# vismaychuriwala/Fast-Image-Editing-with-Generative-Models

Measured on AMD Instinct MI355X. Metric: PIE-Bench images/sec @1024^2 SSD-1B fp16 4-step, higher is better.
Workload: dtype f16

## Files before the change

### fast-image-editing-with-generative-models_amd/csrc/conv_halo.hip

```cpp
#include "gemm_common.h"

using namespace fie_gemm;

namespace {

constexpr int HP = 18;
constexpr int HPIECES = (HP * HP + 7) / 8;
constexpr int HALO_B = HPIECES * 1024;
constexpr int HSLOTS = 6;
constexpr int BNH = 128;
constexpr int STH = 3;
constexpr int WSTAGE_B = BNH * 128;
constexpr int WRING_OFF = 0;
constexpr int HALO_OFF = STH * WSTAGE_B;
constexpr int DUMP_OFF = HALO_OFF + 2 * HALO_B;
constexpr int kLdsHalo = DUMP_OFF + 1024;
constexpr int RWH = BNH / 64;

constexpr int n_w(bool last, int t) { return last && t + 2 > 8 ? 0 : RWH; }
constexpr int n_h(bool last, int t) { return !last && t < HSLOTS ? 1 : 0; }
constexpr int n_wait(bool last, int t) { return (t > 0 ? n_h(last, t - 1) : 0) + n_w(last, t) + n_h(last, t); }

template <bool STAMP>
__global__ __launch_bounds__(512) void conv_halo_kernel(GemmArgs p) {
    constexpr int FM = 4, FN = 4, WM = 64, WN = 64;
    extern __shared__ __attribute__((aligned(16))) half_t smem[];
    char* const lds = reinterpret_cast<char*>(smem);

    const int tid = threadIdx.x;
    const int lane = tid & 63;
    const int wave = __builtin_amdgcn_readfirstlane(tid >> 6);
    const int grp = wave >> 2;
    const int wm = wave & 3, wn = wave >> 2;

    const int bid = xcd_remap(blockIdx.x, gridDim.x);
    const int nt = bid % p.nbn, patch = bid / p.nbn;
    const int ppr = p.OW >> 4, ppi = (p.OH >> 4) * ppr;
    const int b = patch / ppi, pr = patch - b * ppi;
    const int py = pr / ppr, px = pr - py * ppr;
    const int y0 = py << 4, x0 = px << 4;
    const int m0 = (b * p.OH + y0) * p.OW + x0, n0 = nt * BNH;

    const int live = p.probe == 1 ? 0 : 1;
    const __amdgpu_buffer_rsrc_t rs_a = buf_rsrc(p.A1, (int)p.a1_bytes * live);
    const __amdgpu_buffer_rsrc_t rs_w = buf_rsrc(p.Wt, (int)p.w_bytes * live);

    unsigned h_off[HSLOTS];
#pragma unroll
    for (int i = 0; i < HSLOTS; ++i) {
        const int q = wave + 8 * i;
        const int pl = q * 8 + (lane >> 3);
        const int hy = pl / HP, hx = pl - hy * HP;
        const int iy = y0 + hy - 1, ix = x0 + hx - 1;
        const bool ok = q < HPIECES && pl < HP * HP && iy >= 0 && iy < p.H && ix >= 0 && ix < p.W;
        const unsigned chunk = (unsigned)((lane & 7) ^ (hx & 7));
        h_off[i] = ok ? ((unsigned)(b * p.H + iy) * (unsigned)p.W + (unsigned)ix) * (unsigned)p.Cin * 2u + chunk * 16u : kOob;
    }
    auto halo_dst = [&](int i, int buf) -> half_t* {
        const int q = wave + 8 * i;
        return reinterpret_cast<half_t*>(lds + (q < HPIECES ? HALO_OFF + buf * HALO_B + q * 1024 : DUMP_OFF));
    };
    const int lr = lane >> 3;
    const unsigned w_base = (unsigned)(n0 + wave * 8 + lr) * (unsigned)p.ldw * 2u + (unsigned)((lane & 7) ^ lr) * 16u;
    const unsigned w_step = 64u * (unsigned)p.ldw * 2u;
    auto issue_w = [&](int stage, unsigned soff) {
#pragma unroll
        for (int i = 0; i < RWH; ++i)
            bload16(rs_w, reinterpret_cast<half_t*>(lds + WRING_OFF + stage * WSTAGE_B + (wave + 8 * i) * 1024), w_base + (unsigned)i * w_step, soff);
    };
    const unsigned cin2 = (unsigned)p.Cin * 2u;

    const int fr = lane & 15, fq = lane >> 4;
    unsigned a_rd[3][2];
#pragma unroll
    for (int kx = 0; kx < 3; ++kx)
#pragma unroll
        for (int kh = 0; kh < 2; ++kh)
            a_rd[kx][kh] = (unsigned)((wm * FM * HP + fr + kx) * 128 + (((kh * 4 + fq) ^ ((fr + kx) & 7)) << 4));
    unsigned w_rd[2];
#pragma unroll
    for (int kh = 0; kh < 2; ++kh) w_rd[kh] = (unsigned)(2 * lds_off(wn * WN + fr, kh * 4 + fq));

    f32x4 acc[FN][FM];
#pragma unroll
    for (int i = 0; i < FN; ++i)
#pragma unroll
        for (int j = 0; j < FM; ++j) acc[i][j] = (f32x4){0.f, 0.f, 0.f, 0.f};

    unsigned seg[8] = {0, 0, 0, 0, 0, 0, 0, 0}, tprev = 0;
    auto stamp = [&](int i) {
        if constexpr (STAMP) {
            __builtin_amdgcn_sched_barrier(0);
            const unsigned t = (unsigned)__builtin_amdgcn_s_memtime();
            seg[i] += t - tprev;
            tprev = t;
            __builtin_amdgcn_sched_barrier(0);
        }
    };
    if constexpr (STAMP) tprev = (unsigned)__builtin_amdgcn_s_memtime();

    const int nchunks = p.Cin / BK;
#pragma unroll
    for (int i = 0; i < HSLOTS; ++i) bload16(rs_a, halo_dst(i, 0), h_off[i], 0u);
    issue_w(0, 0u);
    issue_w(1, nchunks * 9 > 1 ? cin2 : 0u);
    wait_vm_barrier<RWH>();
    if (grp == 1) __builtin_amdgcn_s_barrier();
    stamp(5);

    f16x8 fw[2][FN], fa[2][FM];
    auto kstep = [&](auto lastc, auto tapc, int c, unsigned hb) {
        constexpr bool LAST = decltype(lastc)::value;
        constexpr int T = decltype(tapc)::value;
        constexpr int KY = T / 3, KX = T % 3;
        constexpr int STAGE = T % STH, FILL = (T + 2) % STH;
        if constexpr (n_w(LAST, T) > 0) {
            constexpr int T2 = (T + 2) % 9;
            const int c2 = T + 2 > 8 ? c + 1 : c;
            issue_w(FILL, (unsigned)T2 * cin2 + (unsigned)c2 * (BK * 2));
        }
        if constexpr (n_h(LAST, T) > 0) bload16(rs_a, halo_dst(T, (c + 1) & 1), h_off[T], (unsigned)(c + 1) * (BK * 2));
        stamp(0);
        const char* const hal = lds + HALO_OFF + hb;
        const char* const wst = lds + WRING_OFF + STAGE * WSTAGE_B;
#pragma unroll
        for (int kh = 0; kh < 2; ++kh) {
#pragma unroll
            for (int i = 0; i < FN; ++i) fw[kh][i] = *reinterpret_cast<const f16x8*>(wst + w_rd[kh] + i * 16 * 128);
#pragma unroll
            for (int j = 0; j < FM; ++j) fa[kh][j] = *reinterpret_cast<const f16x8*>(hal + a_rd[KX][kh] + (j + KY) * HP * 128);
        }
        asm volatile("s_waitcnt lgkmcnt(0)" ::: "memory");
        stamp(1);
        wait_vm_barrier<n_wait(LAST, T)>();
        stamp(2);
        __builtin_amdgcn_sched_barrier(0);
        __builtin_amdgcn_s_setprio(1);
#pragma unroll
        for (int kh = 0; kh < 2; ++kh)
#pragma unroll
            for (int i = 0; i < FN; ++i)
#pragma unroll
                for (int j = 0; j < FM; ++j) acc[i][j] = __builtin_amdgcn_mfma_f32_16x16x32_f16(fw[kh][i], fa[kh][j], acc[i][j], 0, 0, 0);
        __builtin_amdgcn_s_setprio(0);
        __builtin_amdgcn_sched_barrier(0);
        stamp(3);
        __builtin_amdgcn_s_barrier();
        stamp(4);
    };
    auto chunk = [&](auto lastc, int c) {
        const unsigned hb = (c & 1) ? (unsigned)HALO_B : 0u;
        kstep(lastc, std::integral_constant<int, 0>{}, c, hb);
        kstep(lastc, std::integral_constant<int, 1>{}, c, hb);
        kstep(lastc, std::integral_constant<int, 2>{}, c, hb);
        kstep(lastc, std::integral_constant<int, 3>{}, c, hb);
        kstep(lastc, std::integral_constant<int, 4>{}, c, hb);
        kstep(lastc, std::integral_constant<int, 5>{}, c, hb);
        kstep(lastc, std::integral_constant<int, 6>{}, c, hb);
        kstep(lastc, std::integral_constant<int, 7>{}, c, hb);
        kstep(lastc, std::integral_constant<int, 8>{}, c, hb);
    };
    for (int c = 0; c + 1 < nchunks; ++c) chunk(std::false_type{}, c);
    chunk(std::true_type{}, nchunks - 1);
    if (grp == 0) __builtin_amdgcn_s_barrier();

    epilogue<FM, FN, WM, WN, true, true>(p, acc, m0, n0, wm, wn, lane);
    if constexpr (STAMP) {
        asm volatile("s_waitcnt vmcnt(0)" ::: "memory");
        stamp(6);
        if (p.stamps && lane == 0) {
#pragma unroll
            for (int i = 0; i < 8; ++i) p.stamps[((size_t)bid * 8 + wave) * 8 + i] = seg[i];
        }
    }
}


constexpr int K_FIRST = 0, K_MID = 1, K_LAST_F = 2, K_LAST_N = 3, K_LASTREG_S = 4;
constexpr int n2_w(int kind, int t) { return kind == K_LAST_N && t + 2 > 8 ? 0 : RWH; }
constexpr int n2_h(int kind, int t) { return kind != K_LAST_N && t < HSLOTS ? 1 : 0; }
constexpr int n2_st(int var, int kind, int t) { return kind == K_FIRST && t < 8 ? ((var & 2) ? 1 : 2) : 0; }
constexpr int n2_tail(bool res, int kind, int t) { return n2_h(kind, t); }
constexpr int n2_wait(int var, bool res, int kind, int t) {
    return (t > 0 ? n2_tail(res, kind, t - 1) : 0) + ((var & 8) ? 0 : n2_w(kind, t) + n2_tail(res, kind, t));
}
static_assert(n2_tail(true, K_LAST_F, 8) == 0 && n2_tail(true, K_FIRST, 8) == 0 && n2_st(0, K_FIRST, 8) == 0, "tap 8 carries nothing behind its weights");

template <bool RES, bool GN, bool RB, int VAR, bool STAMP, bool SIDE = false, bool GNA = false, bool EDGE = false>
__global__ __launch_bounds__(512) void conv_halo2_kernel(GemmArgs p) {
    constexpr int FM = 4, FN = 4, WN = 64;
    constexpr bool ST16 = (VAR & 2) != 0, STM = (VAR & 4) != 0, IM = (VAR & 8) != 0;
    constexpr bool DEFER = ST16 && STM && !IM;
    static_assert(!(SIDE && (RES || RB)), "1x1 side inputs belong to a resnet's conv2 + shortcut: no residual, no row bias");
    static_assert(!EDGE || (ST16 && !GN && !GNA), "edge patches: 16-byte stores, no GroupNorm sums");
    extern __shared__ __attribute__((aligned(16))) half_t smem[];
    char* const lds = reinterpret_cast<char*>(smem);

    const int tid = threadIdx.x;
// ... 606 lines not shown
                    asm volatile("s_nop 1\n\tv_permlane16_swap_b32 %0, %1" : "+v"(v[0]), "+v"(v[2]));
                    asm volatile("s_nop 1\n\tv_permlane16_swap_b32 %0, %1" : "+v"(v[1]), "+v"(v[3]));
                }
                __builtin_amdgcn_raw_buffer_store_b128(v, rs_c, edge_off(ro_prev + (unsigned)(2 * jj) * c_jstep + (unsigned)(i * 32), 2 * jj), 0, 0);
            }
    } else {
#pragma unroll
        for (int j = 0; j < FM; ++j)
#pragma unroll
            for (int i = 0; i < FN; ++i) __builtin_amdgcn_raw_buffer_store_b64(outp[i][j], rs_c, ro_prev + (unsigned)j * c_jstep + (unsigned)(i * 32), 0, 0);
    }
    if constexpr (STAMP) {
        asm volatile("s_waitcnt vmcnt(0)" ::: "memory");
        stamp(6);
        if (p.stamps && lane == 0) {
#pragma unroll
            for (int i = 0; i < 8; ++i) p.stamps[((size_t)bid * 8 + wave) * 12 + i] = seg[i];
#pragma unroll
            for (int i = 0; i < 4; ++i) p.stamps[((size_t)bid * 8 + wave) * 12 + 8 + i] = kseg[i];
        }
    }
}

template <bool RES, bool GN, bool RB, int VAR, bool STAMP, bool SIDE = false, bool GNA = false, bool EDGE = false>
hipError_t halo2_attr() {
    return hipFuncSetAttribute(reinterpret_cast<const void*>(&conv_halo2_kernel<RES, GN, RB, VAR, STAMP, SIDE, GNA, EDGE>), hipFuncAttributeMaxDynamicSharedMemorySize, kLdsHalo);
}

}

int fie_conv_halo_init(void) {
    hipError_t e = hipFuncSetAttribute(reinterpret_cast<const void*>(&conv_halo_kernel<false>), hipFuncAttributeMaxDynamicSharedMemorySize, kLdsHalo);
    if (e == hipSuccess) e = hipFuncSetAttribute(reinterpret_cast<const void*>(&conv_halo_kernel<true>), hipFuncAttributeMaxDynamicSharedMemorySize, kLdsHalo);
    if (e == hipSuccess) e = halo2_attr<false, false, false, 6, false>();
    if (e == hipSuccess) e = halo2_attr<false, true, false, 6, false>();
    if (e == hipSuccess) e = halo2_attr<true, false, false, 6, false>();
    if (e == hipSuccess) e = halo2_attr<true, true, false, 6, false>();
    if (e == hipSuccess) e = halo2_attr<false, false, true, 6, false>();
    if (e == hipSuccess) e = halo2_attr<false, true, true, 6, false>();
    if (e == hipSuccess) e = halo2_attr<false, false, false, 0, false>();
    if (e == hipSuccess) e = halo2_attr<false, true, false, 0, false>();
    if (e == hipSuccess) e = halo2_attr<true, false, false, 0, false>();
    if (e == hipSuccess) e = halo2_attr<true, true, false, 0, false>();
    if (e == hipSuccess) e = halo2_attr<false, false, true, 0, false>();
    if (e == hipSuccess) e = halo2_attr<false, true, true, 0, false>();
    if (e == hipSuccess) e = halo2_attr<false, false, false, 6, true>();
    if (e == hipSuccess) e = hipFuncSetAttribute(reinterpret_cast<const void*>(&conv_halo2_kernel<false, false, false, 6, false, true>), hipFuncAttributeMaxDynamicSharedMemorySize, kLdsHalo);
    if (e == hipSuccess) e = hipFuncSetAttribute(reinterpret_cast<const void*>(&conv_halo2_kernel<false, true, false, 6, false, true>), hipFuncAttributeMaxDynamicSharedMemorySize, kLdsHalo);
    if (e == hipSuccess) e = halo2_attr<true, true, false, 6, true>();
    if (e == hipSuccess) e = hipFuncSetAttribute(reinterpret_cast<const void*>(&conv_halo2_kernel<false, true, false, 6, false, false, true>), hipFuncAttributeMaxDynamicSharedMemorySize, kLdsHalo + 8192);
    if (e == hipSuccess) e = hipFuncSetAttribute(reinterpret_cast<const void*>(&conv_halo2_kernel<true, true, false, 6, false, false, true>), hipFuncAttributeMaxDynamicSharedMemorySize, kLdsHalo + 8192);
    if (e == hipSuccess) e = halo2_attr<false, false, false, 6, false, false, false, true>();
    if (e == hipSuccess) e = halo2_attr<true, false, false, 6, false, false, false, true>();
    if (e == hipSuccess) e = halo2_attr<false, false, true, 6, false, false, false, true>();
    if (e == hipSuccess) e = halo2_attr<false, false, false, 6, false, true, false, true>();
    if (e != hipSuccess) {
        fie_set_error("conv_halo: hipFuncSetAttribute failed: %s", hipGetErrorString(e));
        return FIE_EHIP;
    }
    return FIE_OK;
}

bool fie_conv_halo_ok(const GemmArgs& a) {
    const bool base = a.stride == 1 && !a.ups && !a.taps2 && !a.oscat && a.pt == 1 && a.pl == 1 && a.H == a.OH && a.W == a.OW && a.OH % 16 == 0 &&
                      a.OW % 16 == 0 && a.Cin % BK == 0 && a.Cin >= BK && !a.w_scale && !a.out_f8 && a.splitk <= 1;
    if (!base) return false;
    if (!a.A2) return !a.A3 && a.K == 9 * a.Cin;
    return a.C2x % BK == 0 && a.C3x % BK == 0 && a.C2x > 0 && (a.A3 != nullptr) == (a.C3x > 0) && a.K == 9 * a.Cin + a.C2x + a.C3x && a.Cin >= 2 * BK && a.N % BNH == 0 &&
           !a.res && !a.rowbias && a.act == FIE_ACT_NONE && a.scale == 1.f && a.lda2 * 2 * (int64_t)a.OW * a.OH < (1ll << 31) && a.lda3 * 2 * (int64_t)a.OW * a.OH < (1ll << 31);
}

bool fie_conv_halo_edge_ok(const GemmArgs& a) {
    const bool base = a.stride == 1 && !a.ups && !a.taps2 && !a.oscat && a.pt == 1 && a.pl == 1 && a.H == a.OH && a.W == a.OW && a.OH > 0 && a.OW > 0 &&
                      (a.OH % 16 != 0 || a.OW % 16 != 0) && a.M % (a.OH * a.OW) == 0 && a.Cin % BK == 0 && a.Cin >= 2 * BK && !a.w_scale && !a.out_f8 &&
                      a.splitk <= 1 && a.N % 64 == 0 && a.ldc >= a.N && !a.gn_partial && !a.gna_tab && a.act == FIE_ACT_NONE && a.scale == 1.f && !(a.rowbias && a.res);
    if (!base) return false;
    if (!a.A2) return !a.A3 && a.K == 9 * a.Cin;
    return a.C2x % BK == 0 && a.C3x % BK == 0 && a.C2x > 0 && (a.A3 != nullptr) == (a.C3x > 0) && a.K == 9 * a.Cin + a.C2x + a.C3x && !a.res && !a.rowbias &&
           a.lda2 * 2 * (int64_t)a.OW * a.OH < (1ll << 31) && a.lda3 * 2 * (int64_t)a.OW * a.OH < (1ll << 31);
}

int64_t fie_conv_halo_patches(const GemmArgs& a) {
    if (a.OH <= 0 || a.OW <= 0) return 0;
    return (int64_t)(a.M / (a.OH * a.OW)) * ((a.OH + 15) / 16) * ((a.OW + 15) / 16);
}

bool fie_conv_halo_gna_ok(const GemmArgs& a) {
    if (!fie_conv_halo_ok(a) || a.A2 || a.rowbias) return false;
    const int nbn = (a.N + BNH - 1) / BNH;
    return a.M == a.OH * a.OW && a.Cin >= 2 * BK && a.Cin <= 1024 && a.N % BNH == 0 && nbn <= 64 && a.act == FIE_ACT_NONE && a.scale == 1.f && a.gn_partial != nullptr &&
           (a.gn_cg == 4 || a.gn_cg == 8 || a.gn_cg == 16);
}

int fie_launch_conv_halo(fie_ctx* ctx, GemmArgs& a, int variant) {
    if (variant == 6) {
        FIE_REQUIRE(fie_conv_halo_edge_ok(a), "halo-resident conv with edge patches (tile code 78): stride-1 same-size 3x3 conv with H or W %% 16 != 0, Cin %% 64 == 0, "
                    "Cin >= 128, N %% 64 == 0, no activation / scale / GroupNorm sums only");
        a.frag_ld = a.OW;
        a.nbn = (a.N + BNH - 1) / BNH;
        a.nbm = (int)fie_conv_halo_patches(a);
        const int tiles = a.nbm * a.nbn;
        int g = tiles < ctx->num_cus ? tiles : ctx->num_cus;
        g -= g % a.nbn;
        FIE_REQUIRE(g >= a.nbn && a.nbn <= ctx->num_cus, "halo-resident conv: more column tiles than CUs");
        const dim3 grid((unsigned)g);
        if (a.A2) fie_launch(ctx, (conv_halo2_kernel<false, false, false, 6, false, true, false, true>), grid, dim3(512), kLdsHalo, a);
        else if (a.res) fie_launch(ctx, (conv_halo2_kernel<true, false, false, 6, false, false, false, true>), grid, dim3(512), kLdsHalo, a);
        else if (a.rowbias) fie_launch(ctx, (conv_halo2_kernel<false, false, true, 6, false, false, false, true>), grid, dim3(512), kLdsHalo, a);
        else fie_launch(ctx, (conv_halo2_kernel<false, false, false, 6, false, false, false, true>), grid, dim3(512), kLdsHalo, a);
        FIE_LAUNCH_CHECK();
        return FIE_OK;
    }
    FIE_REQUIRE(fie_conv_halo_ok(a), "halo-resident conv: stride-1 same-size 3x3 conv with H, W %% 16 == 0 and Cin %% 64 == 0 only");
    a.frag_ld = a.OW;
    a.nbn = (a.N + BNH - 1) / BNH;
    a.nbm = (a.M / (a.OH * a.OW)) * (a.OH >> 4) * (a.OW >> 4);
    const int tiles = a.nbm * a.nbn;
    const bool side = a.A2 != nullptr;
    FIE_REQUIRE(!(side && variant != 2), "halo-resident conv: 1x1 side inputs run on tile code 72 only");
    if (a.gna_tab) {
        FIE_REQUIRE(fie_conv_halo_gna_ok(a), "halo-resident conv with the input's GroupNorm applied in LDS: shape or epilogue not built (fie_conv3x3_gn_ok)");
        int g = tiles < ctx->num_cus ? tiles : ctx->num_cus;
        g -= g % a.nbn;
        const int lds_bytes = kLdsHalo + a.Cin * 8;
        if (a.res) fie_launch(ctx, (conv_halo2_kernel<true, true, false, 6, false, false, true>), dim3((unsigned)g), dim3(512), lds_bytes, a);
        else fie_launch(ctx, (conv_halo2_kernel<false, true, false, 6, false, false, true>), dim3((unsigned)g), dim3(512), lds_bytes, a);
        FIE_LAUNCH_CHECK();
        return FIE_OK;
    }
    if (!side && variant >= 2 && tiles <= ctx->num_cus) variant = variant == 4 ? 1 : 0;
    if (!side && variant >= 2 && (a.Cin < 2 * BK || a.N % BNH != 0 || (a.rowbias && a.res) || (variant == 4 && a.rowbias) || a.act != FIE_ACT_NONE || a.scale != 1.f)) variant = variant == 4 ? 1 : 0;
    if (variant < 2) {
        const dim3 grid((unsigned)tiles);
        if (variant == 1) fie_launch(ctx, (conv_halo_kernel<true>), grid, dim3(512), kLdsHalo, a);
        else fie_launch(ctx, (conv_halo_kernel<false>), grid, dim3(512), kLdsHalo, a);
        FIE_LAUNCH_CHECK();
        return FIE_OK;
    }
    int g = tiles < ctx->num_cus ? tiles : ctx->num_cus;
    g -= g % a.nbn;
    FIE_REQUIRE(g >= a.nbn && a.nbn <= ctx->num_cus, "halo-resident conv: more column tiles than CUs");
    const dim3 grid((unsigned)g);
    const bool res = a.res != nullptr, gn = a.gn_partial != nullptr, rb = a.rowbias != nullptr;
    FIE_REQUIRE(!gn || a.gn_cg == 4 || a.gn_cg == 8 || a.gn_cg == 16, "halo-resident conv: GroupNorm sums need 4, 8 or 16 channels per group");
#define FIE_HALO2(RES, GN, RB, VAR, ST) fie_launch(ctx, (conv_halo2_kernel<RES, GN, RB, VAR, ST>), grid, dim3(512), kLdsHalo, a)
#define FIE_HALO2_V(VAR)                                                                   \
    do {                                                                                   \
        if (rb && gn) FIE_HALO2(false, true, true, VAR, false);                            \
        else if (rb) FIE_HALO2(false, false, true, VAR, false);                            \
        else if (res && gn) FIE_HALO2(true, true, false, VAR, false);                      \
        else if (res) FIE_HALO2(true, false, false, VAR, false);                           \
        else if (gn) FIE_HALO2(false, true, false, VAR, false);                            \
// ... 12 lines not shown
```

### fast-image-editing-with-generative-models_amd/csrc/gemm_common.h

```cpp
#pragma once
#include "fie_internal.h"
#include "gemm_addr.h"

namespace fie_gemm {

constexpr int BK = 64;

struct GemmArgs {
    const half_t* A1; int64_t lda1; int K1;
    const half_t* A2; int64_t lda2;
    const half_t* A3; int64_t lda3; int C2x, C3x; int64_t a3_bytes;
    int H, W, Cin, OH, OW, stride, pt, pl, ups;
    const half_t* Wt; int64_t ldw;
    half_t* C; int64_t ldc;
    int M, N, K;
    const half_t* bias;
    const half_t* rowbias; int64_t ld_rowbias; int rows_per_batch;
    const half_t* res; int64_t ldr;
    float scale; int act;
    int nbm, nbn;
    int64_t a1_bytes, a2_bytes, w_bytes;
    int taps2, oscat, opy, opx;
    int64_t w_par_stride;
    int gn_nch, gn_chunk0;
// ... 504 lines not shown
    asm volatile("s_waitcnt vmcnt(0)" ::: "memory");
    __syncthreads();
#pragma unroll
    for (int i = 0; i < FN; ++i)
#pragma unroll
        for (int j = 0; j < FM; ++j) acc[i][j] = (f32x4){0.f, 0.f, 0.f, 0.f};
    for (int s = 0; s < S; ++s) {
        const __amdgpu_buffer_rsrc_t rs = buf_rsrc(base + (size_t)s * kTile, kTile * 4);
        u32x4 v[FN][FM];
#pragma unroll
        for (int i = 0; i < FN; ++i)
#pragma unroll
            for (int j = 0; j < FM; ++j) v[i][j] = __builtin_amdgcn_raw_buffer_load_b128(rs, (unsigned)((i * FM + j) * NW * 64 + tid) * 16u, 0, 16);
#pragma unroll
        for (int i = 0; i < FN; ++i)
#pragma unroll
            for (int j = 0; j < FM; ++j) acc[i][j] += __builtin_bit_cast(f32x4, v[i][j]);
    }
    return true;
}

__device__ __forceinline__ int xcd_remap(int bid, int nwg) {
    const int q = nwg >> 3, r = nwg & 7, xcd = bid & 7;
    return (xcd < r ? xcd * (q + 1) : r * (q + 1) + (xcd - r) * q) + (bid >> 3);
}

}

int fie_launch_gemm8(fie_ctx* ctx, const fie_gemm::GemmArgs& a, int conv, int split);
int fie_gemm8_init(void);
int fie_gemm_init(void);
int fie_launch_conv_halo(fie_ctx* ctx, fie_gemm::GemmArgs& a, int stamped);
bool fie_conv_halo_ok(const fie_gemm::GemmArgs& a);
bool fie_conv_halo_edge_ok(const fie_gemm::GemmArgs& a);
int64_t fie_conv_halo_patches(const fie_gemm::GemmArgs& a);
int fie_launch_conv_thin(fie_ctx* ctx, fie_gemm::GemmArgs& a);
bool fie_conv_thin_ok(const fie_gemm::GemmArgs& a);
bool fie_conv_halo_gna_ok(const fie_gemm::GemmArgs& a);
int fie_conv_halo_init(void);
int fie_launch_gemm_w8(fie_ctx* ctx, const fie_gemm::GemmArgs& a, int conv, int code);
int fie_gemm_w8_init(void);
int fie_launch_gemm_x8(fie_ctx* ctx, const fie_gemm::GemmArgs& a, int code, int conv);
int fie_gemm_x8_init(void);
```

### fast-image-editing-with-generative-models_amd/csrc/gemm_conv.hip

```cpp
#include <algorithm>
#include <cstdio>
#include <cstdlib>
#include <cstring>
#include <utility>

#include "gemm_common.h"
#include "gemm_tiles.h"

using namespace fie_gemm;

namespace {

template <int BM, int BN, int MODE>
__global__ __launch_bounds__(256) void gemm_kernel(GemmArgs p) {
    constexpr int WM = BM / 2, WN = BN / 2;
    constexpr int FM = WM / 16, FN = WN / 16;
    constexpr int RA = BM / 32, RW = BN / 32;
    __shared__ __attribute__((aligned(16))) half_t smem[2 * (BM + BN) * BK];

    const int tid = threadIdx.x;
    const int lane = tid & 63, wave = tid >> 6;
    const int wm = wave & 1, wn = wave >> 1;

    const int bid = xcd_remap(blockIdx.x, gridDim.x);
// ... 548 lines not shown
}
template <int BM, int BN>
constexpr Tile generic_row(int code, int w8, int x8) { return {code, BM, BN, kGeneric, "gemm_kernel", 0, w8, x8, &launch_generic<BM, BN, 0>, &launch_generic<BM, BN, 1>}; }
template <int CONV, int VARIANT>
int launch_phased(fie_ctx* ctx, GemmArgs& a, dim3) { return fie_launch_gemm8(ctx, a, CONV, VARIANT); }
template <int VARIANT>
int launch_halo(fie_ctx* ctx, GemmArgs& a, dim3) { return fie_launch_conv_halo(ctx, a, VARIANT); }
int launch_thin(fie_ctx* ctx, GemmArgs& a, dim3) { return fie_launch_conv_thin(ctx, a); }

constexpr Tile kTiles[] = {
    generic_row<128, 128>(1, 62, 43),
    generic_row<128, 64>(2, 42, 42),
    generic_row<64, 64>(3, 43, 43),
    RingTile<128, 64, 3, 4, kSplitK | kLnFold>::row(42, "gemm3_kernel", 42, 42),
    RingTile<64, 64, 3, 4, kSplitK>::row(43, "gemm3_kernel", 43, 43),
    RingTile<128, 64, 2, 4, kSplitK>::row(44, "gemm3_kernel", 42, 42),
    RingTile<64, 64, 2, 4, kSplitK>::row(46, "gemm3_kernel", 43, 43),
    RingTile<128, 96, 3, 4, kSplitK>::row(47, "gemm3_kernel", 62, 47),
    RingTile<128, 80, 3, 4, kSplitK>::row(48, "gemm3_kernel", 62, 0),
    RingTile<128, 128, 3, 8, kSplitK>::row(51, "gemm3_kernel", 62, 51),
    RingTile<128, 128, 2, 8, kSplitK>::row(52, "gemm3_kernel", 52, 52),
    RingTile<192, 128, 2, 8, kSplitK>::row(54, "gemm3_kernel", 54, 54),
    RingTile<256, 256, 2, 8>::row(61, "gemm3_kernel", 62, 62),
    RingTile<256, 128, 3, 8, kSplitK>::row(62, "gemm3_kernel", 62, 62),
    RingTile<256, 320, 2, 8, kGemmOnly>::row(63, "gemm3_kernel", 62, 63),
    RingTile<256, 320, 2, 8, kGemmOnly | kAlt | kLnFold>::row(64, "gemm3_kernel", 62, 63),
    RingTile<128, 128, 3, 8, kPF | kSplitK>::row(95, "gemm3_kernel+prefetch", 62, 51),
    RingTile<256, 128, 3, 8, kPF | kSplitK | kLnFold>::row(96, "gemm3_kernel+prefetch", 62, 62),
    RingTile<256, 128, 3, 8, kStamps>::row(97, "gemm3_kernel+prefetch", 62, 0),
    RingTile<256, 128, 3, 8, kPF | kStamps>::row(98, "gemm3_kernel+prefetch", 62, 0),
    RingTile<128, 64, 3, 4, kStamps>::row(94, "gemm3_kernel+prefetch", 62, 0),
    {81, 256, 256, kPhased, "gemm8_kernel", 0, 62, 62, &launch_phased<0, 0>, &launch_phased<1, 0>},
    {82, 256, 256, kPhased, "gemm8_kernel", 0, 62, 0, &launch_phased<0, 1>, &launch_phased<1, 1>},
    {71, 256, 128, kHalo, "conv_halo_kernel", 0, 62, 0, nullptr, &launch_halo<0>},
    {73, 256, 128, kHalo, "conv_halo_kernel", kStamps, 62, 0, nullptr, &launch_halo<1>},
    {72, 256, 128, kHalo, "conv_halo2_kernel", 0, 62, 0, nullptr, &launch_halo<2>},
    {74, 256, 128, kHalo, "conv_halo2_kernel", kStamps, 62, 0, nullptr, &launch_halo<4>},
    {76, 256, 128, kHalo, "conv_halo2_kernel", 0, 62, 0, nullptr, &launch_halo<5>},
    {78, 256, 128, kHaloEdge, "conv_halo2_kernel+edge", 0, 62, 0, nullptr, &launch_halo<6>},
    {77, 64, 16, kThin, "conv_thin_kernel", 0, 62, 0, &launch_thin, &launch_thin},
};
constexpr const Tile* find_tile(int code) {
    for (const Tile& t : kTiles)
        if (t.code == code) return &t;
    return nullptr;
}
constexpr bool is_family(int code, Family f) { return find_tile(code) && find_tile(code)->family == f; }

constexpr int kCandF16[] = {43, 46, 42, 44, 51, 52, 54, 96, 81, 63, 47, 48, 64, 72, 78};
constexpr int kCandW8[] = {43, 42, 62, 52, 54};
constexpr int kCandX8[] = {43, 42, 47, 51, 52, 54, 62, 63};
struct SplitCand { int code, per_cu; };
constexpr SplitCand kSplitF16[] = {{96, 1}, {95, 1}, {47, 1}, {54, 2}, {52, 2}};
constexpr SplitCand kSplitX8[] = {{62, 1}, {51, 1}, {47, 1}, {54, 2}, {52, 2}};

template <size_t N>
constexpr bool f8_built(const fie_f8_tile (&built)[N], int code) {
    const Tile* t = find_tile(code);
    for (const fie_f8_tile& b : built)
        if (t && b.code == code && b.bm == t->bm && b.bn == t->bn) return true;
    return false;
}
constexpr int table_error() {
    for (const Tile& t : kTiles) {
        int n = 0;
        for (const Tile& u : kTiles) n += u.code == t.code;
        if (n != 1) return 1;
        if (!f8_built(kFieW8Tiles, t.w8) || (t.x8 && !f8_built(kFieX8Tiles, t.x8))) return 2;
        if ((t.flags & kSplitK) && t.family != kRing) return 3;
        if ((!t.conv && !(t.flags & kGemmOnly)) || (!t.gemm && t.family != kHalo && t.family != kHaloEdge)) return 4;
    }
    for (int c : kCandF16) if (!find_tile(c)) return 5;
    for (int c : kCandW8) if (!f8_built(kFieW8Tiles, c)) return 6;
    for (int c : kCandX8) if (!f8_built(kFieX8Tiles, c)) return 7;
    for (const SplitCand& c : kSplitF16) if (!find_tile(c.code) || !(find_tile(c.code)->flags & kSplitK)) return 8;
    for (const SplitCand& c : kSplitX8) if (!f8_built(kFieX8Tiles, c.code) || !(find_tile(c.code)->flags & kSplitK)) return 9;
    return 0;
}
static_assert(table_error() == 0, "kTiles / candidate lists inconsistent: see table_error for the rule with that number");

template <int MODE>
int heuristic_code(const fie_ctx* ctx, const GemmArgs& a, bool dma_ok) {
    auto blocks = [&](int bm, int bn) { return (int64_t)((a.M + bm - 1) / bm) * ((a.N + bn - 1) / bn); };
    const int64_t cus = ctx->num_cus;
    const int64_t b256 = blocks(256, 256), b62 = blocks(256, 128), b51 = blocks(128, 128), b42 = blocks(128, 64);
    int code;
    if (!dma_ok) {
        code = b42 >= cus ? 2 : 3;
    } else if (MODE == 1 && fie_conv_halo_ok(a) && 4 * (int64_t)(a.M / 256) * ((a.N + 127) / 128) >= 3 * cus && a.C2x + a.C3x <= 4 * BK &&
               std::find(std::begin(ctx->tune_exclude), std::end(ctx->tune_exclude), 72) == std::end(ctx->tune_exclude)) {
        code = 72;
    } else if (MODE == 1 && fie_conv_halo_edge_ok(a) && 4 * fie_conv_halo_patches(a) * ((a.N + 127) / 128) >= 3 * cus && a.C2x + a.C3x <= 4 * BK &&
               std::find(std::begin(ctx->tune_exclude), std::end(ctx->tune_exclude), 78) == std::end(ctx->tune_exclude)) {
        code = 78;
    } else if (MODE == 1) {
        if (!a.A2 && ((b256 >= cus && (a.N % 256 == 0 || (a.N % 128 != 0 && a.K >= 5760))) ||
            (a.N % 256 == 0 && a.K >= 8192 && 2 * b256 >= cus))) code = 81;
        else if (a.N % 128 == 0 && b62 >= 150) code = 96;
        else if (a.N % 128 == 0 && a.K >= 5760 && b51 >= 100) code = 51;
        else if (2 * b42 < 3 * cus) code = 43;
        else code = 42;
    } else if (MODE == 0 && a.N % 320 == 0 && a.N >= 5120 && 4 * blocks(256, 320) >= 3 * cus) {
// ... 4 lines not shown
        code = 96;
    } else if (a.N >= 2048 && a.K >= 1024 && b51 >= cus) {
        code = 51;
    } else if (a.K <= 640 && a.N <= 640) {
        code = 43;
    } else if (b42 >= cus * 7 / 2 || a.K >= 4096 || (a.K >= 1024 && b42 >= cus)) {
        code = 42;
    } else {
        code = 43;
    }
    return code;
}

constexpr int64_t kSkTickets = 4096;

inline int splitk_fit(const fie_ctx* ctx, const GemmArgs& a, const Tile& t, int want) {
    const int bm = t.bm, bn = t.bn;
    if (want <= 1 || !(t.flags & kSplitK) || !ctx->sk_ws || !ctx->splitk_mode || (a.w_scale && a.a_scale == 0.f)) return 1;
    const int64_t tiles = (int64_t)((a.M + bm - 1) / bm) * ((a.N + bn - 1) / bn) * (a.oscat == 2 ? 4 : 1);
    const int nk = (a.K + BK - 1) / BK / (a.a_scale != 0.f ? 2 : 1);
    int s = want;
    while (s > 1 && (nk / s < 4 || tiles > kSkTickets || (int64_t)(kSkTickets * 4 + tiles * s * bm * bn * 4) > ctx->sk_bytes)) --s;
    return s;
}

template <int MODE>
int run_code(fie_ctx* ctx, GemmArgs& a, int code, int order, bool dma_ok, int split = 1) {
    const Tile* t = find_tile(code);
    FIE_REQUIRE(t != nullptr, "unknown tile code %d", code);
    const Family fam = t->family;
    FIE_REQUIRE(fam == kGeneric || fam == kThin || dma_ok, "tile code %d: shape not eligible for the LDS-DMA kernels (operands >= 2 GiB, Cin %% 64 != 0, or A = [A1 | A2] with K1 %% 64 != 0 or K %% 64 != 0)", code);
    FIE_REQUIRE(!(a.taps2 && (fam == kGeneric || a.w_scale)), "tile code %d: the 2x2 parity convs run on the f16 LDS-DMA kernels only", code);
    FIE_REQUIRE(!(MODE == 1 && a.A2 && (fam == kGeneric || fam == kPhased || a.w_scale)), "tile code %d: conv + 1x1 side inputs run on the f16 ring kernels and the halo-resident kernel (72) only", code);
    FIE_REQUIRE(!(fam == kHalo && (MODE != 1 || !dma_ok || !fie_conv_halo_ok(a))), "tile code %d (halo-resident conv): stride-1 same-size 3x3 conv with H, W %% 16 == 0, Cin %% 64 == 0, f16 weights only", code);
    FIE_REQUIRE(!(fam == kHaloEdge && (MODE != 1 || !dma_ok || !fie_conv_halo_edge_ok(a))), "tile code 78 (halo-resident conv, edge patches): stride-1 same-size 3x3 conv with H or W %% 16 != 0, "
                "Cin %% 64 == 0, Cin >= 128, N %% 64 == 0, f16 weights, no activation / scale / GroupNorm sums only");
    if (order < 0) {
        const int64_t nbm = (a.M + t->bm - 1) / t->bm, nbn = (a.N + t->bn - 1) / t->bn;
        const int64_t per_xcd = (nbm * nbn + 7) / 8;
        const double a_tile = (double)t->bm * a.K * 2 * (MODE == 1 ? 1.0 / 9 : 1.0), w_tile = (double)t->bn * a.K * 2;
        auto fabric = [&](int64_t fast, int64_t slow, double fast_tile, double slow_tile) {
            const int64_t rows = (per_xcd + fast - 1) / fast;
            return (double)(rows < slow ? rows : slow) * slow_tile + (double)(per_xcd < fast ? per_xcd : fast) * fast_tile;
        };
        order = fabric(nbm, nbn, a_tile, w_tile) < fabric(nbn, nbm, w_tile, a_tile) ? 1 : 0;
    }
    const bool x8 = a.w_scale && a.a_scale != 0.f;
    if (x8) {
        FIE_REQUIRE(dma_ok && !a.A2 && !a.taps2, "fp8 activations: plain GEMM / 3x3 conv views on the LDS-DMA kernels only");
        FIE_REQUIRE(t->x8 != 0, "tile code %d has no fp8-activation kernel", code);
        t = find_tile(t->x8);
        if (MODE == 1 && (t->flags & kGemmOnly)) t = find_tile(62);
    } else if (a.w_scale) {
        FIE_REQUIRE(dma_ok, "fp8 weights: shape not eligible for the LDS-DMA kernels (operands >= 2 GiB, Cin %% 64 != 0, or A = [A1 | A2] with K1 %% 64 != 0 or K %% 64 != 0)");
        t = find_tile(t->w8);
    }
    code = t->code;
    a.nbm = (a.M + t->bm - 1) / t->bm;
    a.nbn = (a.N + t->bn - 1) / t->bn;
    split = splitk_fit(ctx, a, *t, split);
    a.splitk = split;
    a.sk_tickets = static_cast<unsigned*>(ctx->sk_ws);
    a.sk_slabs = reinterpret_cast<float*>(static_cast<char*>(ctx->sk_ws) + kSkTickets * 4);
    a.order = order;
    a.probe = ctx->gemm_probe;
    a.epi_prefetch = ctx->epi_prefetch;
// ... 29 lines not shown
}

constexpr size_t kFlushBytes = 384u << 20;

template <int MODE>
std::vector<int> tune_candidates(const fie_ctx* ctx, const GemmArgs& a, int guess) {
    static const bool use47 = !(getenv("FIE_TUNE_47") && getenv("FIE_TUNE_47")[0] == '0');
    std::vector<int> out;
    auto blocks = [&](int bm, int bn) { return (int64_t)((a.M + bm - 1) / bm) * ((a.N + bn - 1) / bn); };
    const bool x8 = a.w_scale && a.a_scale != 0.f;
    const int* cand = x8 ? kCandX8 : a.w_scale ? kCandW8 : kCandF16;
    const size_t ncand = x8 ? std::size(kCandX8) : a.w_scale ? std::size(kCandW8) : std::size(kCandF16);
    auto excluded = [&](int c) {
        for (int e : ctx->tune_exclude)
            if (e == c) return e != 0;
        return false;
    };
    for (size_t i = 0; i < ncand; ++i) {
        const int c = cand[i];
        if (c == guess || excluded(c)) continue;
        if ((c == 43 || c == 46) && blocks(64, 64) > 64 * ctx->num_cus) continue;
        if ((c == 81 || c == 96 || c == 62) && 2 * blocks(256, 128) < ctx->num_cus) continue;
        if ((c == 63 || c == 64) && (MODE != 0 || a.N % 320 != 0 || 2 * blocks(256, 320) < ctx->num_cus)) continue;
        if (c == 47 && !use47) continue;
        if (c == 48 && (a.N % 80 != 0 || blocks(128, 80) > 2 * ctx->num_cus)) continue;
        if (x8 && MODE == 1 && c == 63) continue;
        if (x8 && (c == 62 || c == 51) && 2 * blocks(c == 62 ? 256 : 128, 128) < ctx->num_cus) continue;
        if (c == 81 && MODE == 1 && a.A2) continue;
        if (c == 72 && (MODE != 1 || !fie_conv_halo_ok(a) || 2 * (int64_t)(a.M / 256) * ((a.N + 127) / 128) < ctx->num_cus)) continue;
        if (c == 78 && (MODE != 1 || !fie_conv_halo_edge_ok(a) || 2 * fie_conv_halo_patches(a) * ((a.N + 127) / 128) < ctx->num_cus)) continue;
        out.push_back(c);
    }
    if ((!a.w_scale || x8) && ctx->sk_ws && ctx->splitk_mode && !excluded(10000)) {
        for (const SplitCand& c : x8 ? kSplitX8 : kSplitF16) {
            if (excluded(c.code)) continue;
            const Tile& t = *find_tile(c.code);
            const int64_t nb = blocks(t.bm, t.bn) * (a.oscat == 2 ? 4 : 1);
            if (nb >= ctx->num_cus * c.per_cu) continue;
            for (int sp = 2; sp <= 4; ++sp) {
                if (nb * sp > (int64_t)ctx->num_cus * c.per_cu * 21 / 20) break;
                if (splitk_fit(ctx, a, t, sp) != sp) continue;
                out.push_back(c.code + 10000 * sp);
            }
        }
    }
    return out;
}

template <int MODE>
int autotune(fie_ctx* ctx, GemmArgs& a, int guess, bool dma_ok) {
    const size_t bytes = (size_t)a.M * (a.oscat ? 4 : 1) * (size_t)a.ldc * sizeof(half_t);
    if (bytes > ctx->tune_bytes) {
        if (ctx->tune_buf) (void)hipFree(ctx->tune_buf);
        ctx->tune_buf = nullptr;
        ctx->tune_bytes = 0;
        if (hipMalloc(&ctx->tune_buf, bytes) != hipSuccess) { (void)hipGetLastError(); return guess; }
        ctx->tune_bytes = bytes;
    }
    if (!ctx->tune_flush && hipMalloc(&ctx->tune_flush, kFlushBytes) != hipSuccess) { (void)hipGetLastError(); ctx->tune_flush = nullptr; return guess; }
    hipEvent_t e0, e1;
    if (hipEventCreate(&e0) != hipSuccess || hipEventCreate(&e1) != hipSuccess) return guess;
    (void)hipDeviceSynchronize();
    GemmArgs t = a;
    t.C = static_cast<half_t*>(ctx->tune_buf);
    auto time_of = [&](int code, int split = 1) -> float {
        float ms[7];
        for (int rep = -1; rep < 7; ++rep) {
            (void)hipMemsetAsync(ctx->tune_flush, rep & 1, kFlushBytes, ctx->stream);
            if ((size_t)a.a1_bytes <= kFlushBytes) (void)hipMemcpyAsync(ctx->tune_flush, a.A1, (size_t)a.a1_bytes, hipMemcpyDeviceToDevice, ctx->stream);
            if (a.A2 && a.A2 != a.A1 && (size_t)a.a2_bytes <= kFlushBytes) (void)hipMemcpyAsync(ctx->tune_flush, a.A2, (size_t)a.a2_bytes, hipMemcpyDeviceToDevice, ctx->stream);
            (void)hipEventRecord(e0, ctx->stream);
            if (run_code<MODE>(ctx, t, code, -1, dma_ok, split) != FIE_OK) return 1e30f;
            (void)hipEventRecord(e1, ctx->stream);
            if (hipEventSynchronize(e1) != hipSuccess) return 1e30f;
// ... 52 lines not shown
        const fie_tile_override& o = ctx->overrides[i];
        if (o.mode == (MODE == 1) && o.M == a.M && o.N == a.N && o.K == a.K) { decode(o.code); pinned = true; }
    }
    if (ctx->force_tile) { decode(ctx->force_tile); pinned = true; }
    const fie_tune_key key{MODE, a.M, a.N, a.K, a.K1, MODE == 1 ? a.stride * 2 + a.ups + 8 * a.taps2 + 16 * (a.A2 != nullptr) + 32 * (a.A3 != nullptr) : 0, a.w_scale == nullptr ? 0 : a.a_scale != 0.f ? 2 : 1};
    auto note_candidates = [&](int rule, const std::vector<int>& cands) {
        char line[256];
        int n = snprintf(line, sizeof(line), "%s M=%d N=%d K=%d K1=%d geom=%d w8=%d rule=%d cands=", MODE == 1 ? "conv" : "gemm", key.M, key.N, key.K, key.K1, key.geom, key.w8, rule);
        for (size_t i = 0; i < cands.size() && n < (int)sizeof(line) - 8; ++i) n += snprintf(line + n, sizeof(line) - n, i ? ",%d" : "%d", cands[i]);
        ctx->tune_cands->push_back(line);
    };
    if (MODE == 1 && !pinned && !ctx->gemm_probe && fie_conv_thin_ok(a) && a.M >= 131072 &&
        std::find(std::begin(ctx->tune_exclude), std::end(ctx->tune_exclude), 77) == std::end(ctx->tune_exclude)) {
        if (ctx->tune_cands) note_candidates(77, {});
        return run_code<MODE>(ctx, a, 77, 0, dma_ok, 1);
    }
    if (ctx->tune_cands && !pinned && !ctx->gemm_probe) {
        note_candidates(code, dma_ok ? tune_candidates<MODE>(ctx, a, code) : std::vector<int>{});
        return run_code<MODE>(ctx, a, code, order, dma_ok, split);
    }
    if (ctx->autotune && !pinned && dma_ok && !ctx->gemm_probe) {
        auto it = ctx->tuned.find(key);
        if (it != ctx->tuned.end()) {
            decode(it->second);
        } else if (ctx->autotune == 1 && !ctx->recording) {
            hipStreamCaptureStatus cap = hipStreamCaptureStatusNone;
            if (hipStreamIsCapturing(ctx->stream, &cap) == hipSuccess && cap == hipStreamCaptureStatusNone) {
                const int best = autotune<MODE>(ctx, a, code, dma_ok);
                ctx->tuned[key] = best;
                decode(best);
            }
        }
    }
    if (MODE == 1 && !pinned && ((is_family(code, kHalo) && !fie_conv_halo_ok(a)) || (is_family(code, kHaloEdge) && !fie_conv_halo_edge_ok(a)))) {
        code = heuristic_code<MODE>(ctx, a, dma_ok);
        order = -1;
        split = 1;
    }
    return run_code<MODE>(ctx, a, code, order, dma_ok, split);
}

int check_epilogue(const char* who, int N, int64_t ldc, const void* res, int64_t ldr, int act) {
    FIE_REQUIRE(act >= FIE_ACT_NONE && act <= FIE_ACT_GEGLU, "%s: unknown act %d", who, act);
    FIE_REQUIRE(N % 4 == 0, "%s: N=%d must be a multiple of 4", who, N);
    FIE_REQUIRE(ldc % 4 == 0 || act == FIE_ACT_GEGLU, "%s: ldc=%lld must be a multiple of 4", who, (long long)ldc);
    FIE_REQUIRE(!res || ldr % 4 == 0, "%s: ldr=%lld must be a multiple of 4", who, (long long)ldr);
    FIE_REQUIRE(!(res && act == FIE_ACT_GEGLU), "%s: GEGLU epilogue takes no residual", who);
    return FIE_OK;
}

__global__ void pack_rows_kernel(const half_t* src, int64_t ld_src, int N, int K, half_t* dst, int64_t ldw, int Npad,
                                 int interleave2) {
    const int64_t total = (int64_t)Npad * ldw;
    for (int64_t i = blockIdx.x * (int64_t)blockDim.x + threadIdx.x; i < total; i += (int64_t)gridDim.x * blockDim.x) {
        const int n = (int)(i / ldw), k = (int)(i - (int64_t)n * ldw);
        half_t v = (half_t)0.f;
        if (n < N && k < K) {
            const int sn = interleave2 ? ((n & 1) ? (N / 2 + (n >> 1)) : (n >> 1)) : n;
            v = src[(int64_t)sn * ld_src + k];
        }
        dst[i] = v;
    }
}

__global__ void pack_conv_kernel(const half_t* src, int Cout, int Cin, int cin_pad, half_t* dst, int64_t ldw, int Npad) {
    const int64_t total = (int64_t)Npad * ldw;
    for (int64_t i = blockIdx.x * (int64_t)blockDim.x + threadIdx.x; i < total; i += (int64_t)gridDim.x * blockDim.x) {
// ... 440 lines not shown
```

Measured before the change: 15.22.

## Add split-K variant of halo-resident 3x3 conv kernel for small grids

After: 15.00. 1.4% lower.

```diff
diff --git a/fast-image-editing-with-generative-models_amd/csrc/conv_halo.hip b/fast-image-editing-with-generative-models_amd/csrc/conv_halo.hip
--- a/fast-image-editing-with-generative-models_amd/csrc/conv_halo.hip
+++ b/fast-image-editing-with-generative-models_amd/csrc/conv_halo.hip
@@ -21,8 +21,9 @@
 constexpr int n_h(bool last, int t) { return !last && t < HSLOTS ? 1 : 0; }
 constexpr int n_wait(bool last, int t) { return (t > 0 ? n_h(last, t - 1) : 0) + n_w(last, t) + n_h(last, t); }
 
-template <bool STAMP>
+template <bool STAMP, bool SPLIT = false>
 __global__ __launch_bounds__(512) void conv_halo_kernel(GemmArgs p) {
+    static_assert(!(STAMP && SPLIT), "the stamped instantiation does not split");
     constexpr int FM = 4, FN = 4, WM = 64, WN = 64;
     extern __shared__ __attribute__((aligned(16))) half_t smem[];
     char* const lds = reinterpret_cast<char*>(smem);
@@ -34,7 +35,9 @@
     const int wm = wave & 3, wn = wave >> 2;
 
     const int bid = xcd_remap(blockIdx.x, gridDim.x);
-    const int nt = bid % p.nbn, patch = bid / p.nbn;
+    const int nsplit = SPLIT ? p.splitk : 1;
+    const int tile = bid / nsplit, slice = bid - tile * nsplit;
+    const int nt = tile % p.nbn, patch = tile / p.nbn;
     const int ppr = p.OW >> 4, ppi = (p.OH >> 4) * ppr;
     const int b = patch / ppi, pr = patch - b * ppi;
     const int py = pr / ppr, px = pr - py * ppr;
@@ -100,16 +103,19 @@
     if constexpr (STAMP) tprev = (unsigned)__builtin_amdgcn_s_memtime();
 
     const int nchunks = p.Cin / BK;
-#pragma unroll
-    for (int i = 0; i < HSLOTS; ++i) bload16(rs_a, halo_dst(i, 0), h_off[i], 0u);
-    issue_w(0, 0u);
-    issue_w(1, nchunks * 9 > 1 ? cin2 : 0u);
+    const int c0 = SPLIT ? slice * (nchunks / nsplit) + min(slice, nchunks % nsplit) : 0;
+    const int c1 = SPLIT ? c0 + nchunks / nsplit + (slice < nchunks % nsplit ? 1 : 0) : nchunks;
+    const unsigned k0 = (unsigned)c0 * (BK * 2);
+#pragma unroll
+    for (int i = 0; i < HSLOTS; ++i) bload16(rs_a, halo_dst(i, 0), h_off[i], k0);
+    issue_w(0, k0);
+    issue_w(1, cin2 + k0);
     wait_vm_barrier<RWH>();
     if (grp == 1) __builtin_amdgcn_s_barrier();
     stamp(5);
 
     f16x8 fw[2][FN], fa[2][FM];
-    auto kstep = [&](auto lastc, auto tapc, int c, unsigned hb) {
+    auto kstep = [&](auto lastc, auto tapc, int c, unsigned hb, int nbuf) {
         constexpr bool LAST = decltype(lastc)::value;
         constexpr int T = decltype(tapc)::value;
         constexpr int KY = T / 3, KX = T % 3;
@@ -119,7 +125,7 @@
             const int c2 = T + 2 > 8 ? c + 1 : c;
             issue_w(FILL, (unsigned)T2 * cin2 + (unsigned)c2 * (BK * 2));
         }
-        if constexpr (n_h(LAST, T) > 0) bload16(rs_a, halo_dst(T, (c + 1) & 1), h_off[T], (unsigned)(c + 1) * (BK * 2));
+        if constexpr (n_h(LAST, T) > 0) bload16(rs_a, halo_dst(T, nbuf), h_off[T], (unsigned)(c + 1) * (BK * 2));
         stamp(0);
         const char* const hal = lds + HALO_OFF + hb;
         const char* const wst = lds + WRING_OFF + STAGE * WSTAGE_B;
@@ -149,21 +155,26 @@
         stamp(4);
     };
     auto chunk = [&](auto lastc, int c) {
-        const unsigned hb = (c & 1) ? (unsigned)HALO_B : 0u;
-        kstep(lastc, std::integral_constant<int, 0>{}, c, hb);
-        kstep(lastc, std::integral_constant<int, 1>{}, c, hb);
-        kstep(lastc, std::integral_constant<int, 2>{}, c, hb);
-        kstep(lastc, std::integral_constant<int, 3>{}, c, hb);
-        kstep(lastc, std::integral_constant<int, 4>{}, c, hb);
-        kstep(lastc, std::integral_constant<int, 5>{}, c, hb);
-        kstep(lastc, std::integral_constant<int, 6>{}, c, hb);
-        kstep(lastc, std::integral_constant<int, 7>{}, c, hb);
-        kstep(lastc, std::integral_constant<int, 8>{}, c, hb);
-    };
-    for (int c = 0; c + 1 < nchunks; ++c) chunk(std::false_type{}, c);
-    chunk(std::true_type{}, nchunks - 1);
+        const int par = (c - c0) & 1;
+        const unsigned hb = par ? (unsigned)HALO_B : 0u;
+        const int nbuf = par ^ 1;
+        kstep(lastc, std::integral_constant<int, 0>{}, c, hb, nbuf);
+        kstep(lastc, std::integral_constant<int, 1>{}, c, hb, nbuf);
+        kstep(lastc, std::integral_constant<int, 2>{}, c, hb, nbuf);
+        kstep(lastc, std::integral_constant<int, 3>{}, c, hb, nbuf);
+        kstep(lastc, std::integral_constant<int, 4>{}, c, hb, nbuf);
+        kstep(lastc, std::integral_constant<int, 5>{}, c, hb, nbuf);
+        kstep(lastc, std::integral_constant<int, 6>{}, c, hb, nbuf);
+        kstep(lastc, std::integral_constant<int, 7>{}, c, hb, nbuf);
+        kstep(lastc, std::integral_constant<int, 8>{}, c, hb, nbuf);
+    };
+    for (int c = c0; c + 1 < c1; ++c) chunk(std::false_type{}, c);
+    chunk(std::true_type{}, c1 - 1);
     if (grp == 0) __builtin_amdgcn_s_barrier();
 
+    if constexpr (SPLIT) {
+        if (!splitk_reduce<FM, FN, 8>(p, acc, tile, slice, tid, lds)) return;
+    }
     epilogue<FM, FN, WM, WN, true, true>(p, acc, m0, n0, wm, wn, lane);
     if constexpr (STAMP) {
         asm volatile("s_waitcnt vmcnt(0)" ::: "memory");
@@ -836,6 +847,7 @@
 int fie_conv_halo_init(void) {
     hipError_t e = hipFuncSetAttribute(reinterpret_cast<const void*>(&conv_halo_kernel<false>), hipFuncAttributeMaxDynamicSharedMemorySize, kLdsHalo);
     if (e == hipSuccess) e = hipFuncSetAttribute(reinterpret_cast<const void*>(&conv_halo_kernel<true>), hipFuncAttributeMaxDynamicSharedMemorySize, kLdsHalo);
+    if (e == hipSuccess) e = hipFuncSetAttribute(reinterpret_cast<const void*>(&conv_halo_kernel<false, true>), hipFuncAttributeMaxDynamicSharedMemorySize, kLdsHalo);
     if (e == hipSuccess) e = halo2_attr<false, false, false, 6, false>();
     if (e == hipSuccess) e = halo2_attr<false, true, false, 6, false>();
     if (e == hipSuccess) e = halo2_attr<true, false, false, 6, false>();
@@ -867,11 +879,20 @@
 
 bool fie_conv_halo_ok(const GemmArgs& a) {
     const bool base = a.stride == 1 && !a.ups && !a.taps2 && !a.oscat && a.pt == 1 && a.pl == 1 && a.H == a.OH && a.W == a.OW && a.OH % 16 == 0 &&
-                      a.OW % 16 == 0 && a.Cin % BK == 0 && a.Cin >= BK && !a.w_scale && !a.out_f8 && a.splitk <= 1;
+                      a.OW % 16 == 0 && a.Cin % BK == 0 && a.Cin >= BK && !a.w_scale && !a.out_f8;
     if (!base) return false;
+    if (a.splitk > 1 && (a.A2 || a.A3 || a.gna_tab || a.Cin / BK < a.splitk)) return false;
     if (!a.A2) return !a.A3 && a.K == 9 * a.Cin;
     return a.C2x % BK == 0 && a.C3x % BK == 0 && a.C2x > 0 && (a.A3 != nullptr) == (a.C3x > 0) && a.K == 9 * a.Cin + a.C2x + a.C3x && a.Cin >= 2 * BK && a.N % BNH == 0 &&
            !a.res && !a.rowbias && a.act == FIE_ACT_NONE && a.scale == 1.f && a.lda2 * 2 * (int64_t)a.OW * a.OH < (1ll << 31) && a.lda3 * 2 * (int64_t)a.OW * a.OH < (1ll << 31);
+}
+
+bool fie_conv_halo_split_ok(const fie_ctx* ctx, const GemmArgs& a, int s) {
+    GemmArgs t = a;
+    t.splitk = s;
+    if (s <= 1 || !fie_conv_halo_ok(t)) return false;
+    const int64_t tiles = (int64_t)(a.M / (a.OH * a.OW)) * (a.OH >> 4) * (a.OW >> 4) * ((a.N + BNH - 1) / BNH);
+    return tiles * s <= (int64_t)ctx->num_cus * 21 / 20;
 }
 
 bool fie_conv_halo_edge_ok(const GemmArgs& a) {
@@ -922,6 +943,14 @@
     const int tiles = a.nbm * a.nbn;
     const bool side = a.A2 != nullptr;
     FIE_REQUIRE(!(side && variant != 2), "halo-resident conv: 1x1 side inputs run on tile code 72 only");
+    if (a.splitk > 1) {
+        FIE_REQUIRE(variant == 0, "halo-resident conv: split-K runs on tile code 71 only");
+        FIE_REQUIRE(fie_conv_halo_split_ok(ctx, a, a.splitk) && a.sk_slabs && a.sk_tickets, "halo-resident conv: split-K %d needs a plain conv (no 1x1 side inputs, no GroupNorm of the input) "
+                    "with at least %d 64-channel chunks, a grid of tiles x %d within the chip and a bound split-K workspace", a.splitk, a.splitk, a.splitk);
+        fie_launch(ctx, (conv_halo_kernel<false, true>), dim3((unsigned)(tiles * a.splitk)), dim3(512), kLdsHalo, a);
+        FIE_LAUNCH_CHECK();
+        return FIE_OK;
+    }
     if (a.gna_tab) {
         FIE_REQUIRE(fie_conv_halo_gna_ok(a), "halo-resident conv with the input's GroupNorm applied in LDS: shape or epilogue not built (fie_conv3x3_gn_ok)");
         int g = tiles < ctx->num_cus ? tiles : ctx->num_cus;
diff --git a/fast-image-editing-with-generative-models_amd/csrc/gemm_common.h b/fast-image-editing-with-generative-models_amd/csrc/gemm_common.h
--- a/fast-image-editing-with-generative-models_amd/csrc/gemm_common.h
+++ b/fast-image-editing-with-generative-models_amd/csrc/gemm_common.h
@@ -560,6 +560,7 @@
 int fie_gemm_init(void);
 int fie_launch_conv_halo(fie_ctx* ctx, fie_gemm::GemmArgs& a, int stamped);
 bool fie_conv_halo_ok(const fie_gemm::GemmArgs& a);
+bool fie_conv_halo_split_ok(const fie_ctx* ctx, const fie_gemm::GemmArgs& a, int s);
 bool fie_conv_halo_edge_ok(const fie_gemm::GemmArgs& a);
 int64_t fie_conv_halo_patches(const fie_gemm::GemmArgs& a);
 int fie_launch_conv_thin(fie_ctx* ctx, fie_gemm::GemmArgs& a);
diff --git a/fast-image-editing-with-generative-models_amd/csrc/gemm_conv.hip b/fast-image-editing-with-generative-models_amd/csrc/gemm_conv.hip
--- a/fast-image-editing-with-generative-models_amd/csrc/gemm_conv.hip
+++ b/fast-image-editing-with-generative-models_amd/csrc/gemm_conv.hip
@@ -604,7 +604,7 @@
     RingTile<128, 64, 3, 4, kStamps>::row(94, "gemm3_kernel+prefetch", 62, 0),
     {81, 256, 256, kPhased, "gemm8_kernel", 0, 62, 62, &launch_phased<0, 0>, &launch_phased<1, 0>},
     {82, 256, 256, kPhased, "gemm8_kernel", 0, 62, 0, &launch_phased<0, 1>, &launch_phased<1, 1>},
-    {71, 256, 128, kHalo, "conv_halo_kernel", 0, 62, 0, nullptr, &launch_halo<0>},
+    {71, 256, 128, kHalo, "conv_halo_kernel", kSplitK, 62, 0, nullptr, &launch_halo<0>},
     {73, 256, 128, kHalo, "conv_halo_kernel", kStamps, 62, 0, nullptr, &launch_halo<1>},
     {72, 256, 128, kHalo, "conv_halo2_kernel", 0, 62, 0, nullptr, &launch_halo<2>},
     {74, 256, 128, kHalo, "conv_halo2_kernel", kStamps, 62, 0, nullptr, &launch_halo<4>},
@@ -623,7 +623,7 @@
 constexpr int kCandW8[] = {43, 42, 62, 52, 54};
 constexpr int kCandX8[] = {43, 42, 47, 51, 52, 54, 62, 63};
 struct SplitCand { int code, per_cu; };
-constexpr SplitCand kSplitF16[] = {{96, 1}, {95, 1}, {47, 1}, {54, 2}, {52, 2}};
+constexpr SplitCand kSplitF16[] = {{96, 1}, {95, 1}, {47, 1}, {54, 2}, {52, 2}, {71, 1}};
 constexpr SplitCand kSplitX8[] = {{62, 1}, {51, 1}, {47, 1}, {54, 2}, {52, 2}};
 
 template <size_t N>
@@ -639,7 +639,7 @@
         for (const Tile& u : kTiles) n += u.code == t.code;
         if (n != 1) return 1;
         if (!f8_built(kFieW8Tiles, t.w8) || (t.x8 && !f8_built(kFieX8Tiles, t.x8))) return 2;
-        if ((t.flags & kSplitK) && t.family != kRing) return 3;
+        if ((t.flags & kSplitK) && t.family != kRing && t.code != 71) return 3;
         if ((!t.conv && !(t.flags & kGemmOnly)) || (!t.gemm && t.family != kHalo && t.family != kHaloEdge)) return 4;
     }
     for (int c : kCandF16) if (!find_tile(c)) return 5;
@@ -710,6 +710,10 @@
     FIE_REQUIRE(fam == kGeneric || fam == kThin || dma_ok, "tile code %d: shape not eligible for the LDS-DMA kernels (operands >= 2 GiB, Cin %% 64 != 0, or A = [A1 | A2] with K1 %% 64 != 0 or K %% 64 != 0)", code);
     FIE_REQUIRE(!(a.taps2 && (fam == kGeneric || a.w_scale)), "tile code %d: the 2x2 parity convs run on the f16 LDS-DMA kernels only", code);
     FIE_REQUIRE(!(MODE == 1 && a.A2 && (fam == kGeneric || fam == kPhased || a.w_scale)), "tile code %d: conv + 1x1 side inputs run on the f16 ring kernels and the halo-resident kernel (72) only", code);
+    a.splitk = (fam == kHalo || fam == kHaloEdge) ? split : 1;
+    FIE_REQUIRE(!((fam == kHalo || fam == kHaloEdge) && split > 1 && (MODE != 1 || !dma_ok || !(t->flags & kSplitK) || !fie_conv_halo_split_ok(ctx, a, split) || splitk_fit(ctx, a, *t, split) != split)),
+                "tile code %d (halo-resident conv) with split-K %d: code 71 only, on a plain conv (no 1x1 side inputs) with at least %d 64-channel chunks, tiles x %d within the chip "
+                "and the split-K workspace bound and large enough", code, split, split, split);
     FIE_REQUIRE(!(fam == kHalo && (MODE != 1 || !dma_ok || !fie_conv_halo_ok(a))), "tile code %d (halo-resident conv): stride-1 same-size 3x3 conv with H, W %% 16 == 0, Cin %% 64 == 0, f16 weights only", code);
     FIE_REQUIRE(!(fam == kHaloEdge && (MODE != 1 || !dma_ok || !fie_conv_halo_edge_ok(a))), "tile code 78 (halo-resident conv, edge patches): stride-1 same-size 3x3 conv with H or W %% 16 != 0, "
                 "Cin %% 64 == 0, Cin >= 128, N %% 64 == 0, f16 weights, no activation / scale / GroupNorm sums only");
@@ -805,7 +809,10 @@
         out.push_back(c);
     }
     if ((!a.w_scale || x8) && ctx->sk_ws && ctx->splitk_mode && !excluded(10000)) {
-        for (const SplitCand& c : x8 ? kSplitX8 : kSplitF16) {
+        const SplitCand* const sc = x8 ? kSplitX8 : kSplitF16;
+        const size_t nsc = x8 ? std::size(kSplitX8) : std::size(kSplitF16);
+        for (size_t ci = 0; ci < nsc; ++ci) {
+            const SplitCand& c = sc[ci];
             if (excluded(c.code)) continue;
             const Tile& t = *find_tile(c.code);
             const int64_t nb = blocks(t.bm, t.bn) * (a.oscat == 2 ? 4 : 1);
@@ -813,6 +820,7 @@
             for (int sp = 2; sp <= 4; ++sp) {
                 if (nb * sp > (int64_t)ctx->num_cus * c.per_cu * 21 / 20) break;
                 if (splitk_fit(ctx, a, t, sp) != sp) continue;
+                if (t.family == kHalo && (MODE != 1 || !fie_conv_halo_split_ok(ctx, a, sp))) continue;
                 out.push_back(c.code + 10000 * sp);
             }
         }
@@ -931,7 +939,7 @@
             }
         }
     }
-    if (MODE == 1 && !pinned && ((is_family(code, kHalo) && !fie_conv_halo_ok(a)) || (is_family(code, kHaloEdge) && !fie_conv_halo_edge_ok(a)))) {
+    if (MODE == 1 && !pinned && ((is_family(code, kHalo) && (!fie_conv_halo_ok(a) || (split > 1 && (!fie_conv_halo_split_ok(ctx, a, split) || splitk_fit(ctx, a, *find_tile(code), split) != split)))) || (is_family(code, kHaloEdge) && !fie_conv_halo_edge_ok(a)))) {
         code = heuristic_code<MODE>(ctx, a, dma_ok);
         order = -1;
         split = 1;
```
